# ivario123/r7020e-visual-odometry

Measured on AMD Instinct MI355X. Metric: stereo frames/sec @1242x375 (SIFT detect+describe x2 + stereo matchFeatures), higher is better.
Workload: dtype f32 (i8 MFMA for exact descriptor dot products); 1 GPU; BASELINE configs[1]: SIFT detect+describe + BF match on 1242x375 synthetic stereo, ~2k keypoints/image; rows=375, cols=1242, parallelism=frames sharded over 1 GPU(s)

## Files before the change

__graft_entry__.py:

```python
import os
import subprocess
import sys
from pathlib import Path

ROOT = Path(__file__).resolve().parent
PKG = ROOT / "r7020e-visual-odometry_amd"


def build() -> None:
    env = dict(os.environ)
    env.setdefault("ARCH", "gfx950")
    jobs = str(min(8, os.cpu_count() or 4))
    subprocess.run(["make", "-s", "-j", jobs, "-C", str(PKG / "csrc")], check=True, env=env)
    subprocess.run(["make", "-s", "-C", str(ROOT / "oracle")], check=True, env=env)
    subprocess.run(["make", "-s", "-C", str(ROOT / "tests" / "mex_shim")], check=True, env=env)
    subprocess.run(["make", "-s", "-C", str(ROOT / "tests" / "describe_ref")], check=True, env=env)
    subprocess.run(["make", "-s", "-C", str(ROOT / "tests" / "tri_quality_ref")], check=True, env=env)
    subprocess.run(["make", "-s", "-C", str(ROOT / "tests" / "pose_refine_ref")], check=True, env=env)
    sys.path.insert(0, str(ROOT))
    import vo_amd
    from r7020e_visual_odometry_amd import vo
    lib = vo.load_library()
    missing = [s for s in vo.EXPORTS if not hasattr(lib, s)]
    if missing:
        raise RuntimeError(f"libvo.so is missing exports: {missing}")


def smoke() -> None:
    import numpy as np
    sys.path.insert(0, str(ROOT))
    sys.path.insert(0, str(ROOT / "oracle"))
    import torch
    import vo_amd
    from r7020e_visual_odometry_amd import vo, synthetic as syn
    import oracle

    assert torch.cuda.is_available(), "smoke() needs an MI355X"
    L, R = syn.stereo_pair(syn.SEED_BASE + 1)
    ctx = vo.Context(375, 1242, 1, device=0)
    dl = torch.from_numpy(L[None]).cuda()
    dr = torch.from_numpy(R[None]).cuda()
# ... 21 lines not shown
```

r7020e-visual-odometry_amd/csrc/blur_plan.h:

```cpp
#pragma once

namespace vo {

#define VO_BLUR_RADII(X) X(5) X(6) X(8) X(10) X(13)

constexpr bool blur_radius_tabled(int r)
{
#define VO_BLUR_IS_R(RR) || r == RR
    return false VO_BLUR_RADII(VO_BLUR_IS_R);
#undef VO_BLUR_IS_R
}

constexpr int kTagLevel = 0;
constexpr int kTagBase = 1;
constexpr int kTagBaseU8 = kTagBase | 4;
constexpr int kTagCachedStores = 2;
constexpr int kTagNoRowPass = 8;
constexpr int kTagNoColPass = 16;
constexpr int kTagNoLds = 32;
constexpr int kTagNoHalo = 64;

#define BS_P 4

constexpr int bs_rh(int r, int cpl) { return (r + cpl - 1) / cpl * cpl; }
// ... 14 lines not shown

constexpr int blur_bands(int R, int th) { return (R + th - 1) / th; }
constexpr int blur_grid_strips(int C, int r, int cpl, int tag) { return (C + bs_sw(r, cpl, tag) - 1) / bs_sw(r, cpl, tag); }

constexpr BlurPlan blur_plan(BlurRole role, int R, int C, int n_img, int r)
{
    constexpr int kMaxTH = 128, kWaveTarget = 2048, kCpl2MaxC = 1400, kU8MinRows = 64;
    const bool base = role != BlurRole::Level;
    const int cpl = (!base && C <= kCpl2MaxC) ? 2 : 4;
    const int tag = role == BlurRole::BaseU8 ? kTagBaseU8 : base ? kTagBase : kTagLevel;
    const long waves_rows = (long)R * ((C + 64 * cpl - 1) / (64 * cpl)) * n_img / kWaveTarget;
    const long cap = base && kBaseMaxTH < kMaxTH ? kBaseMaxTH : kMaxTH;
    int th = (int)(waves_rows < cap ? waves_rows : cap) / BS_P * BS_P;
    if (th < BS_P) th = BS_P;
    BlurPlan p{role, false, 0, 0, 0, 0, 0, !base && waves_rows >= kMaxTH};
    if (!blur_radius_tabled(r) || R < th || R <= r + BS_P + 2 || (role == BlurRole::BaseU8 && R < kU8MinRows)) return p;
    p.streamed = true;
    p.cpl = cpl; p.tag = tag; p.th = th;
    p.n_bands = blur_bands(R, th);
    p.n_strips = blur_grid_strips(C, r, cpl, tag);
    return p;
}

}
```

r7020e-visual-odometry_amd/csrc/sift.hip:

```cpp
#include "vo_internal.h"
#include "blur_plan.h"
#include <cstdlib>
#include <cstring>
#include <cmath>
#include <algorithm>
#include <utility>
#include <type_traits>
#include <mutex>

namespace vo {

struct Kern { float k[VO_SIFT_MAX_RADIUS + 1]; int r; float* nb; int nb_pitch, nb_rows, nb_cols; };

static int desc_radius_cap(const Pyramid& py, const vo_sift_params& p);

void build_pyramid_geometry(Pyramid& py, int rows, int cols, int n_img, const vo_sift_params& p)
{
    memset(&py, 0, sizeof(py));
    const int L = p.n_octave_layers;
    py.L = L;
    py.n_img = n_img;
    py.n_oct = vo_num_octaves(rows, cols, p.upsample);
    int R = p.upsample ? rows * 2 : rows, C = p.upsample ? cols * 2 : cols;
    size_t off = 0;
    size_t tmp_plane = 0;
    for (int o = 0; o < py.n_oct; ++o) {
        OctGeom& g = py.oct[o];
        if (o) { R /= 2; C /= 2; }
        g.rows = R; g.cols = C;
        g.dmax = (int)sqrt((double)C * C + (double)R * R);
        g.pitch = (C + 255) / 256 * 256;
        g.plane = (size_t)g.rows * g.pitch;
        for (int i = 0; i < L + 3; ++i) { g.g_off[i] = off; off += g.plane; }
        if (g.plane > tmp_plane) tmp_plane = g.plane;
    }
    py.istride = off;
    py.total = off * n_img;
    py.tmp_plane = tmp_plane;
    double sig[VO_SIFT_MAX_LAYERS];
    vo_level_sigmas(L, p.sigma, sig);
    py.krad[0] = vo_gauss_kernel(vo_base_sigma(p.sigma, p.upsample), py.kern[0], VO_SIFT_MAX_RADIUS + 1);
    for (int i = 1; i < L + 3; ++i) py.krad[i] = vo_gauss_kernel(sig[i], py.kern[i], VO_SIFT_MAX_RADIUS + 1);
    int w = 0, b = 0, t = 0;
    for (int o = 0; o < py.n_oct; ++o) {
        int ir = py.oct[o].rows - 2 * VO_SIFT_BORDER, ic = py.oct[o].cols - 2 * VO_SIFT_BORDER;
        if (ir < 0) ir = 0;
        if (ic < 0) ic = 0;
        py.wrow[o] = ic > 0 ? ((py.oct[o].cols - VO_SIFT_BORDER - 1) / 64 + 2) / 2 * 2 : 0;
        for (int l = 0; l < L; ++l) { py.wbase[b++] = w; w += ir * py.wrow[o]; }
        py.ebase[o] = t;
        py.estrips[o] = py.wrow[o] / 2;
        t += py.estrips[o] * ((ir + VO_EXT_BAND - 1) / VO_EXT_BAND);
    }
    py.wbase[b] = w;
    py.n_words = w;
    py.ebase[py.n_oct] = t;
    py.n_units = t;
    py.n_seg = (w + VO_SEG_WORDS - 1) / VO_SEG_WORDS;
    py.dcap = desc_radius_cap(py, p);
}

SiftBuffers sift_view(const SiftBuffers& b, const Pyramid& py, int img0, int n)
{
    SiftBuffers v = b;
    v.arena = b.arena + (size_t)img0 * py.istride;
    v.tmp = b.tmp + (size_t)img0 * py.tmp_plane;
    v.mask = b.mask + (size_t)img0 * py.n_words;
    v.woff = b.woff + (size_t)img0 * py.n_seg;
    v.cand = b.cand + (size_t)img0 * b.cand_cap;
    v.n_cand = b.n_cand + img0;
    v.acc = b.acc + (size_t)img0 * b.cand_cap;
    v.n_acc = b.n_acc + img0;
    v.cout = b.cout + (size_t)img0 * b.cand_cap;
    v.koff = b.koff + (size_t)img0 * b.cand_cap;
// ... 252 lines not shown
        }
    }
}


struct U8Src { const uint8_t* p; int ld, rows, cols; };
__host__ __device__ constexpr int bs_u8_dw(int r, int cpl) { return ((64 * cpl + 2 * bs_rh(r, cpl)) / 2 + 3 + 3 + 4 + 3) / 4; }
__host__ __device__ constexpr int bs_u8_rows(int r) { return (2 * r + BS_P + kBaseMaxTH) / 2 + 4; }

__device__ __forceinline__ vo_f4 up4_from_words(uint32_t a0, uint32_t a1, uint32_t sa, uint32_t b0, uint32_t b1, uint32_t sb)
{
    const uint32_t ba = __builtin_amdgcn_alignbyte(a1, a0, sa), bb = __builtin_amdgcn_alignbyte(b1, b0, sb);
    float r[4];
#pragma unroll
    for (int i = 0; i < 4; ++i) {
        const uint32_t xa = 1 + (i >> 1), xb = (i & 1) ? xa + 1 : xa - 1;
        const uint32_t sel = xa | xb << 8 | (4 + xa) << 16 | (4 + xb) << 24;
        const uint32_t q = __builtin_amdgcn_perm(bb, ba, sel);
        r[i] = (float)__builtin_amdgcn_udot4(q, 0x01030309u, 0u, false) * 0.0625f;
    }
    return vo_f4{r[0], r[1], r[2], r[3]};
}

template <int RAD, bool EDGE, int TAG, int CPL>
__device__ __forceinline__ void blur_stream_body(const float* __restrict__ sp, int pitch, int R, int C,
                                                 float* __restrict__ g_out, const Kern& K,
                                                 int x0, int y0, int TH, float* rb, const U8Src& u8,
                                                 float* __restrict__ nbo, uint32_t* __restrict__ stg)
{
    typedef float vec_t __attribute__((ext_vector_type(CPL)));
    constexpr bool UP = (TAG & 4) != 0;
    static_assert(!UP || CPL == 4, "the fused x2 upsample uses 4 columns per lane");
    constexpr bool XCH = bs_hl(RAD, CPL, TAG);
    constexpr int SW = 64 * CPL;
    constexpr int P = BS_P;
    constexpr int RH = bs_rh(RAD, CPL);
    constexpr int NQ = 1 + 2 * RH / CPL;
    constexpr int NP = CPL / 2;
    constexpr int NR = 2 * RAD + P;
    constexpr int F = (2 * RAD + P - 1) / P * P;
    constexpr int E = F - 2 * RAD;
    constexpr int RW = bs_rw(RAD, CPL);
    if constexpr ((TAG & 4) != 0) {
        if (TH > kBaseMaxTH) return;
    }
    const int lane = threadIdx.x;
    const int xl = x0 - (XCH ? RH : 0) + CPL * lane;
    const bool hl = lane < RH / CPL, hr = !hl && lane < 2 * RH / CPL;
    const int hx = XCH ? xl : hl ? x0 - RH + CPL * lane : hr ? x0 + SW + CPL * (lane - RH / CPL) : x0 - RH;
    const int hpos = hl ? CPL * lane : hr ? RH + SW + CPL * (lane - RH / CPL) : -1;
    float* const dummy = rb + RW + CPL * lane;
// ... 36 lines not shown
#pragma unroll
            for (int q = 0; q < SCH; ++q) {
                const int t = t0 + 64 * q + lane;
                const int row = t / SWD, k = t - row * SWD;
                const uint32_t ro = delta + (uint32_t)(sr0 + row) * (uint32_t)u8.ld + (uint32_t)s_lo;
                v[q] = (uint32_t)__builtin_amdgcn_raw_buffer_load_b32(rs_in, t < total ? (ro & ~3u) + 4u * (uint32_t)k : 0x80000000u, 0, 0);
            }
#pragma unroll
            for (int q = 0; q < SCH; ++q)
                if (t0 + 64 * q + lane < total) stg[t0 + 64 * q + lane] = v[q];
        }
        __syncthreads();
    }
    auto s_off = [&](int y, int x) {
        return (y - sr0) * (4 * SWD) + (x - s_lo) + (int)((delta + (uint32_t)y * (uint32_t)u8.ld + (uint32_t)s_lo) & 3u);
    };
    const uint8_t* const stg8 = reinterpret_cast<const uint8_t*>(stg);

    constexpr int NSET = XCH ? 2 : 1;
    vec_t pf[NSET * P], ph[NSET * P];
    typedef uint32_t u2_t __attribute__((ext_vector_type(2)));
    u2_t pw[UP && !EDGE ? NSET * P : 1][4];
    vo_f2 H[NR][NP];
    const int gm = (xl >> 1) - 1, gh = (hx >> 1) - 1;

    auto gather = [&](const float* rowp, const int* idx) {
        vec_t v;
#pragma unroll
        for (int i = 0; i < CPL; ++i) v[i] = rowp[idx[i]];
        return v;
    };

    auto yref = [&](int kk) {
        const int p = y0 - RAD - E + kk;
        if constexpr (XCH) return p < 0 ? -p : (p >= R ? 2 * R - 2 - p : p);
        else return vo_reflect101(p, R);
    };
    auto s_words = [&](int y, int x) {
        const int o = s_off(y, x);
        const uint32_t* w = stg + (o >> 2);
        return u2_t{w[0], w[1]};
    };
#define VO_BS_LOAD(KK, SL)                                                                        \
    do {                                                                                          \
        const int yin_ = yref(KK);                                                                \
        if constexpr (UP) {                                                                       \
// ... 117 lines not shown
                const int y = y0 + kk - F;
                const bool act = (!XCH || (lane >= RH / CPL && lane < 64 - RH / CPL)) && xl < C && y < R &&
                                 (MODE == 1 || (kk >= F && kk < F + TH));
                constexpr uint32_t OOB = 0x80000000u;
                const uint32_t vo = act ? (uint32_t)(y * pitch + xl) * 4u : OOB;
                constexpr int AUX = (TAG & 2) ? 0 : 2;
                if constexpr (CPL == 4)
                    __builtin_amdgcn_raw_buffer_store_b128(__builtin_bit_cast(vo_i4, g), rs_out, vo, 0, AUX);
                else
                    __builtin_amdgcn_raw_buffer_store_b64(__builtin_bit_cast(vo_i2, g), rs_out, vo, 0, AUX);
                if constexpr ((u & 1) == 0 && !(TAG & 1)) {
                    const int yn = y >> 1, c0 = xl >> 1;
                    const bool rowok = act && yn < K.nb_rows;
                    const uint32_t nbase = (uint32_t)(yn * K.nb_pitch + c0) * 4u;
                    const float g0 = g[0];
                    __builtin_amdgcn_raw_buffer_store_b32(__float_as_int(g0), rs_nb, rowok && c0 < K.nb_cols ? nbase : OOB,
                                                          0, 0);
                    if constexpr (CPL == 4) {
                        const float g2 = g[2];
                        __builtin_amdgcn_raw_buffer_store_b32(__float_as_int(g2), rs_nb,
                                                              rowok && c0 + 1 < K.nb_cols ? nbase + 4u : OOB, 0, 0);
                    }
                }
            }
            if constexpr (!XCH) __syncthreads();
        });
#pragma unroll
        for (int q = 0; q < 2 * RAD; ++q)
#pragma unroll
            for (int c = 0; c < NP; ++c) H[q][c] = H[q + P][c];
    };

    vo_static_for<P>([&](auto uc) { VO_BS_LOAD(decltype(uc)::value, decltype(uc)::value); });
    using I0 = std::integral_constant<int, 0>;
    using I1 = std::integral_constant<int, 1>;
    using I2 = std::integral_constant<int, 2>;
    if constexpr (NSET == 1) {
#pragma unroll 1
        for (int kk0 = 0; kk0 < F; kk0 += P) block(kk0, I0{}, I0{});
#pragma unroll 1
        for (int kk0 = F; kk0 < F + TH; kk0 += P) block(kk0, I1{}, I0{});
    } else {
#pragma unroll 1
        for (int kk0 = 0; kk0 < F + TH; kk0 += 2 * P) {
            block(kk0, I2{}, I0{});
            block(kk0 + P, I2{}, I1{});
        }
    }
#undef VO_BS_LOAD
}

#ifndef VO_BLUR_OCC3_MAXR
#define VO_BLUR_OCC3_MAXR 6
#endif
#ifndef VO_BASE_WAVES
#define VO_BASE_WAVES 3
// ... 6 lines not shown
    vo_ss_prio();
    constexpr int RH = bs_rh(RAD, CPL), SW = bs_sw(RAD, CPL, TAG);
    constexpr bool XCH = bs_hl(RAD, CPL, TAG);
    __shared__ __attribute__((aligned(16))) float rb[XCH ? 4 : bs_rw(RAD, CPL) + 64 * CPL];
    __shared__ uint32_t stg[(TAG & 4) ? bs_u8_rows(RAD) * bs_u8_dw(RAD, CPL) : 1];
    const int bid = xcd_remap(blockIdx.x, gridDim.x);
    const int strip = bid % n_strips, tb = bid / n_strips;
    const int band = tb % n_bands, img = tb / n_bands;
    const int x0 = strip * SW, y0 = band * TH;
    const int THb = min(TH, (R - y0 + BS_P - 1) / BS_P * BS_P);
    const size_t os = img * splane, od = img * dplane;
    U8Src u8{nullptr, 0, in_rows, in_cols};
    int margin = 0;
    if (TAG & 4) {
        u8.p = ((img & 1) ? isrc.right : isrc.left) + (size_t)(img >> 1) * isrc.frame_stride;
        u8.ld = isrc.ld;
        margin = 16;
    }
    float* const nbo = K.nb ? K.nb + od : nullptr;
    if (x0 - RH < 0 || (XCH ? x0 - RH + 64 * CPL : x0 + SW + RH) + margin > C)
        blur_stream_body<RAD, true, TAG, CPL>(src + os, pitch, R, C, g_out + od, K, x0, y0, THb, rb, u8, nbo, stg);
    else
        blur_stream_body<RAD, false, TAG, CPL>(src + os, pitch, R, C, g_out + od, K, x0, y0, THb, rb, u8, nbo, stg);
}

__global__ __launch_bounds__(256) void k_down(const float* __restrict__ src, size_t splane, int spitch,
                                              float* __restrict__ dst, size_t dplane, int dpitch, int C)
{
    const int x = blockIdx.x * 256 + threadIdx.x, y = blockIdx.y, img = blockIdx.z;
    if (x < C) dst[img * dplane + (size_t)y * dpitch + x] = src[img * splane + (size_t)(2 * y) * spitch + 2 * x];
}

#ifndef VO_SMALL_PX
#define VO_SMALL_PX 9216
#endif
#ifndef VO_SMALL_T
#define VO_SMALL_T 1024
#endif

constexpr int SMV = 8;
template <int RAD>
__device__ __forceinline__ void small_pass(const float* __restrict__ src, float* __restrict__ dst, float* __restrict__ gdst,
                                           int gpitch, int R, int C, bool rows, const float* __restrict__ kk,
                                           const int* __restrict__ tab, int tid)
{
    const int len = rows ? C : R, other = rows ? R : C, runs = (len + SMV - 1) / SMV;
// ... 351 lines not shown
    uint32_t cnt = 0;
#pragma unroll
    for (int q = 0; q < 4; ++q) {
        mw[q] = (w0 + q < nw) ? m[w0 + q] : 0ull;
        cnt += (uint32_t)__popcll(mw[q]);
    }
#pragma unroll
    for (int q = 0; q < 4; q += 2) {
        const unsigned long long ev = mw[q], od = mw[q + 1];
        mw[q] = vo_spread32((uint32_t)ev) | vo_spread32((uint32_t)od) << 1;
        mw[q + 1] = vo_spread32((uint32_t)(ev >> 32)) | vo_spread32((uint32_t)(od >> 32)) << 1;
    }
    uint32_t idx = segoff[(size_t)img * py->n_seg + seg] + block_exscan_256(cnt, sh);
    if (!cnt) return;
#pragma unroll
    for (int q = 0; q < 4; ++q) {
        unsigned long long mm = mw[q];
        if (!mm) continue;
        int o, layer, r, k;
        decode_word(py, w0 + q, o, layer, r, k);
        while (mm) {
            const int bit = __ffsll((long long)mm) - 1;
            mm &= mm - 1;
            if (idx < (uint32_t)cand_cap) cand[(size_t)img * cand_cap + idx] = pack_cand(o, layer, r, 64 * k + bit);
            idx++;
        }
    }
}

template <typename T>
__device__ __forceinline__ T wave_tree_sum(T v)
{
    auto bits = [](T x) { return __builtin_bit_cast(int, x); };
    auto val = [](int x) { return __builtin_bit_cast(T, x); };
    v = v + val(__builtin_amdgcn_permlane32_swap(bits(v), bits(v), false, false)[1]);
    v = v + val(__builtin_amdgcn_permlane16_swap(bits(v), bits(v), false, false)[1]);
    v = v + val(__builtin_amdgcn_update_dpp(0, bits(v), 0x108, 0xF, 0xF, true));
    v = v + val(__builtin_amdgcn_update_dpp(0, bits(v), 0x104, 0xF, 0xF, true));
    v = v + val(__builtin_amdgcn_update_dpp(0, bits(v), 0x102, 0xF, 0xF, true));
    v = v + val(__builtin_amdgcn_update_dpp(0, bits(v), 0x101, 0xF, 0xF, true));
    return val(__builtin_amdgcn_readlane(bits(v), 0));
}
__device__ __forceinline__ float wave_max(float v)
{
    auto bits = [](float x) { return __float_as_int(x); };
    v = fmaxf(v, __int_as_float(__builtin_amdgcn_permlane32_swap(bits(v), bits(v), false, false)[1]));
    v = fmaxf(v, __int_as_float(__builtin_amdgcn_permlane16_swap(bits(v), bits(v), false, false)[1]));
// ... 812 lines not shown
    const size_t lds = sizeof(float) * ft_lds_floats(K.r);
    if (lds > 64 * 1024) raise_lds_limit((const void*)k_blur_fused<RAD>);
    VO_LAUNCH_NAMED("k_blur_fused", (k_blur_fused<RAD>), dim3((C + FT_W - 1) / FT_W, (R + FT_H - 1) / FT_H, n_img), dim3(256), lds, s,
                    src, plane, dplane, pitch, R, C, g, K);
}

static void launch_blur(const BlurPlan& pl, int n_img, hipStream_t s, const float* src, size_t plane, size_t dplane, int pitch,
                        int R, int C, float* g, const Kern& K, const ImageSrc& isrc, int in_rows, int in_cols)
{
    switch (K.r) {
#define VO_BLUR_CASE(RR) \
    case RR: return launch_blur_r<RR>(pl, n_img, s, src, plane, dplane, pitch, R, C, g, K, isrc, in_rows, in_cols);
        VO_BLUR_RADII(VO_BLUR_CASE)
#undef VO_BLUR_CASE
    default: return launch_blur_r<0>(pl, n_img, s, src, plane, dplane, pitch, R, C, g, K, isrc, in_rows, in_cols);
    }
}

static float ext_threshold(const Pyramid& py, const vo_sift_params& p)
{
    return (float)floor(0.5 * p.contrast_threshold / py.L * 255.0);
}

struct SmallPlan { int o_small, rtab, cap, bcap; size_t lds; };
static SmallPlan small_plan(const Pyramid& py)
{
    SmallPlan sp{py.n_oct, 0, 0, 0, 0};
    int maxr = 0;
    for (int i = 1; i < py.L + 3; ++i) maxr = std::max(maxr, py.krad[i]);
    for (int o = py.n_oct - 1; o >= 1; --o) {
        int rt = 0, ct = 0, cap = 0, bcap = 0;
        bool fits = true;
        for (int q = o; q < py.n_oct; ++q) {
            fits = fits && py.oct[q].rows * py.oct[q].cols <= VO_SMALL_PX;
            cap = std::max(cap, py.oct[q].rows * py.oct[q].cols);
            if (q > o) bcap = std::max(bcap, py.oct[q].rows * py.oct[q].cols);
            rt = std::max(rt, py.oct[q].rows + 2 * maxr);
            ct = std::max(ct, py.oct[q].cols + 2 * maxr);
        }
        cap = (cap + 3) & ~3;
        bcap = (bcap + 3) & ~3;
        const size_t lds = sizeof(float) * (3 * (size_t)cap + bcap) + sizeof(int) * (rt + ct);
        if (!fits || lds > 160 * 1024) break;
        sp = SmallPlan{o, rt, cap, bcap, lds};
    }
    return sp;
}

int sift_small_octave(const Pyramid& py) { return small_plan(py).o_small; }

void sift_enqueue_small(const Pyramid& py, SiftBuffers& b, int n_img, hipStream_t s, const Pyramid* d_py)
{
    const SmallPlan sp = small_plan(py);
    if (sp.o_small >= py.n_oct) return;

    raise_lds_limit((const void*)k_small_pyr);
    VO_LAUNCH_NAMED("k_blur_small", k_small_pyr, dim3(n_img), dim3(VO_SMALL_T), sp.lds, s, d_py, b.arena, sp.o_small,
                    sp.rtab, sp.cap, sp.bcap);
}

void sift_enqueue_pyramid(const Pyramid& py, SiftBuffers& b, const ImageSrc& src, int n_img, const vo_sift_params& p,
                          hipStream_t s, const Pyramid* d_py, hipEvent_t ev_o0, const ScaleChains& ch)
{
    const int L = py.L;
    float* A = b.arena;
    const SmallPlan sp = small_plan(py);
    const int o_small = sp.o_small;
    const bool forked = ch.down != nullptr && ch.down != s;
    int o_fork = std::min(1, o_small - 1);
    while (o_fork + 1 < o_small &&
           blur_plan(BlurRole::Level, py.oct[o_fork + 1].rows, py.oct[o_fork + 1].cols, n_img, py.krad[1]).full_bands)
        ++o_fork;
    bool base_done = false;
    for (int o = 0; o < py.n_oct; ++o) {
        const OctGeom& g = py.oct[o];
        const int R = g.rows, C = g.cols;
        if (o == o_small) break;
        if (forked && o == o_fork + 1) s = ch.down;
        if (o == 0) {
            const Kern K0 = make_kern(py, 0);
            const int rows = p.upsample ? R / 2 : R, cols = p.upsample ? C / 2 : C;
            BlurPlan pl = blur_plan(p.upsample ? BlurRole::BaseU8 : BlurRole::BaseFloat, R, C, n_img, K0.r);
            const bool from_u8 = pl.role == BlurRole::BaseU8 && pl.streamed;
            if (!from_u8) {
                const dim3 qg((g.pitch / 4 + 255) / 256, R, n_img);
// ... 1 lines not shown
                    VO_LAUNCH(k_base_src<true>, qg, dim3(256), 0, s, src, rows, cols, b.tmp, g.plane, g.pitch, R, C, n_img);
                else
                    VO_LAUNCH(k_base_src<false>, qg, dim3(256), 0, s, src, rows, cols, b.tmp, g.plane, g.pitch, R, C, n_img);
                pl = blur_plan(BlurRole::BaseFloat, R, C, n_img, K0.r);
            }
            launch_blur(pl, n_img, s, from_u8 ? nullptr : b.tmp, from_u8 ? 0 : g.plane, py.istride, g.pitch, R, C,
                        A + g.g_off[0], K0, src, from_u8 ? rows : 0, from_u8 ? cols : 0);
        } else if (!base_done) {
            const OctGeom& pg = py.oct[o - 1];
            VO_LAUNCH(k_down, dim3((C + 255) / 256, R, n_img), dim3(256), 0, s, A + pg.g_off[L], py.istride, pg.pitch,
                      A + g.g_off[0], py.istride, g.pitch, C);
        }
        for (int i = 1; i < L + 3; ++i) {
            Kern K = make_kern(py, i);
            const BlurPlan pl = blur_plan(BlurRole::Level, R, C, n_img, K.r);
            if (i == L) {
                base_done = pl.streamed && o + 1 < o_small;
                if (base_done) {
                    const OctGeom& ng = py.oct[o + 1];
                    K.nb = A + ng.g_off[0];
                    K.nb_pitch = ng.pitch; K.nb_rows = ng.rows; K.nb_cols = ng.cols;
                }
            }
            launch_blur(pl, n_img, s, A + g.g_off[i - 1], py.istride, py.istride, g.pitch, R, C, A + g.g_off[i], K, src, 0, 0);
            if (forked && o == o_fork && i == L) {
                hipEventRecord(ch.ev_fork, s);
                hipStreamWaitEvent(ch.down, ch.ev_fork, 0);
            }
        }
        if (o == 0 && ev_o0) hipEventRecord(ev_o0, s);
    }
}

#ifndef VO_FEATURE_GRID
#define VO_FEATURE_GRID 32768
#endif
constexpr int kFeatureGrid = VO_FEATURE_GRID;

void sift_enqueue_extrema(const Pyramid& py, SiftBuffers& b, int n_img, const vo_sift_params& p, hipStream_t s,
                          const Pyramid* d_py, int o_begin, int o_end)
{
    const int L = py.L;
    float* A = b.arena;
    const float thr = ext_threshold(py, p);
    const int u_first = py.ebase[o_begin], u_last = py.ebase[o_end];
    if (u_last > u_first) {
        const dim3 ge((u_last - u_first) * n_img);
// ... 49 lines not shown
    VO_LAUNCH(k_refine, dim3(VO_REFINE_BLOCKS), dim3(256), 0, s, d_py, A, b.cand, b.n_cand, b.cout, b.acc, b.n_acc, b.koff, b.cand_cap, n_img,
              p.contrast_threshold, p.edge_threshold, p.sigma);
    const size_t fpre_bytes = sizeof(int) * (size_t)(n_img + 1);
    const size_t dt_bytes = sizeof(uint32_t) * (size_t)dt_stride(py.dcap);
    VO_LAUNCH_NAMED("k_orient", (k_orient<36>), dim3(kFeatureGrid), dim3(64), fpre_bytes, s, d_py, A, b.n_acc, b.acc,
                    b.cout, b.koff, b.cand_cap, n_img);
    VO_LAUNCH(k_scan_cands, dim3(n_img), dim3(1024), 0, s, b.cout, b.n_cand, b.koff, b.n_kp, b.cand_cap);
    if (strongest > 0) {
        const dim3 gsel(VO_SEL_BLOCKS, n_img);
        VO_LAUNCH(k_sel_keys, gsel, dim3(VO_SEL_TILE), 0, s, b.cout, b.n_acc, b.acc, b.koff, b.n_kp, b.n_det, b.skey, b.snpk,
                  b.cand_cap);
        VO_LAUNCH(k_sel_rank, gsel, dim3(VO_SEL_TILE), 0, s, b.n_acc, b.acc, b.skey, b.snpk, b.koff, b.n_det, b.n_kp, b.cand_cap,
                  strongest);
    }
    VO_LAUNCH(k_expand, dim3(256), dim3(256), 0, s, b.cout, b.n_acc, b.acc, b.koff, b.kp, b.kpi, b.cand_cap, b.kp_cap,
              n_img, p.upsample, strongest > 0 ? strongest : b.kp_cap);
    VO_LAUNCH_NAMED("k_desc", (k_desc<VO_DESC_COPIES>), dim3(kFeatureGrid), dim3(64), dt_bytes + fpre_bytes, s, d_py, A,
                    b.kpi, b.n_kp, b.desc, b.meta, b.kp_cap, n_img);
}

void sift_enqueue_describe(const Pyramid& py, SiftBuffers& b, const ImageSrc& src, int n_img, int n_points,
                           const vo_sift_params& p, hipStream_t s, const Pyramid* d_py)
{
    sift_enqueue_pyramid(py, b, src, n_img, p, s, d_py);
    sift_enqueue_small(py, b, n_img, s, d_py);
    if (n_points <= 0) return;
    VO_LAUNCH(k_points, dim3(std::min(256, (n_points + 255) / 256)), dim3(256), 0, s, b.kp, b.n_kp, b.kpi, b.kp_cap, n_img,
              p.upsample);
    const size_t fpre_bytes = sizeof(int) * (size_t)(n_img + 1);
    const size_t dt_bytes = sizeof(uint32_t) * (size_t)dt_stride(VO_SIFT_DESCR_RMAX);
    VO_LAUNCH_NAMED("k_desc_pts", (k_desc_pts<VO_DESC_COPIES>), dim3(std::min(kFeatureGrid, n_points)), dim3(64),
                    dt_bytes + fpre_bytes, s, d_py, b.arena, b.kpi, b.n_kp, b.desc, b.meta, b.kp_cap, n_img);
}

void sift_enqueue(const Pyramid& py, SiftBuffers& b, const ImageSrc& src, int n_img, const vo_sift_params& p,
                  hipStream_t s, const Pyramid* d_py, int strongest)
{
    sift_enqueue_pyramid(py, b, src, n_img, p, s, d_py);
    sift_enqueue_pyramid_tail(py, b, n_img, p, s, d_py, 0);
    sift_enqueue_features(py, b, n_img, p, s, d_py, strongest);
}

}
```

r7020e-visual-odometry_amd/csrc/vo_api.hip:

```cpp
#include "vo_internal.h"
#include "vo_geom.h"
#include <climits>
#include <cmath>
#include <cstdio>
#include <cstring>
#include <cstdarg>
#include <string>
#include <vector>
#include <deque>
#include <algorithm>

namespace vo {

Profiler* g_prof = nullptr;

void Profiler::begin(const char* name, hipStream_t s)
{
    if (used + 2 > (int)pool.size()) {
        int add = std::max(64, (int)pool.size());
        for (int i = 0; i < add; ++i) { hipEvent_t e; hipEventCreate(&e); pool.push_back(e); }
    }
    marks.push_back({name, used});
    hipEventRecord(pool[used], s);
    used += 1;
// ... 984 lines not shown
                U[k].cam = c->ud_cam[k];
                U[k].in = k ? pr : pl;
                U[k].out = c->d_rect + ((size_t)k * c->max_batch + f0) * fs;
                U[k].copy = c->ud_on[k] ? 0 : 1;
                U[k].pad = 0;
            }
            undistort_launch(U, 2, c->rows, c->cols, nf, fs, fs, sp);
            pl = U[0].out;
            pr = U[1].out;
        }
        ImageSrc src{pl, pr, fs, c->cols, 0};
        SiftBuffers v = sift_view(S.sb, c->py, 2 * f0, 2 * nf);
        ScaleChains ch;
        ch.down = sd;
        ch.ev_fork = c->ev_down[p];
        sift_enqueue_pyramid(c->py, v, src, 2 * nf, c->sp, sp, c->d_py, c->ev_o0[p], ch);
        HIPC(c, hipEventRecord(c->ev_top[p], sp));
        sift_enqueue_small(c->py, v, 2 * nf, sd, c->d_py);
        HIPC(c, hipEventRecord(c->ev_join[p], sd));
    }
    for (int p = 0; p < parts; ++p) {
        const int f0 = B * p / parts, nf = B * (p + 1) / parts - f0;
        SiftBuffers v = sift_view(S.sb, c->py, 2 * f0, 2 * nf);
        HIPC(c, hipStreamWaitEvent(st, iso ? c->ev_join[p] : c->ev_o0[p], 0));
        sift_enqueue_extrema(c->py, v, 2 * nf, c->sp, st, c->d_py, 0, 1);
        HIPC(c, hipStreamWaitEvent(st, c->ev_top[p], 0));
        HIPC(c, hipStreamWaitEvent(st, c->ev_join[p], 0));
        sift_enqueue_extrema(c->py, v, 2 * nf, c->sp, st, c->d_py, 1, o_small);
        sift_enqueue_extrema(c->py, v, 2 * nf, c->sp, st, c->d_py, o_small, c->py.n_oct);
        sift_enqueue_features(c->py, v, 2 * nf, c->sp, st, c->d_py, c->strongest);
        if (p == parts - 1) HIPC(c, hipEventRecord(S.ev_arena, st));
        match_launch(match_view(S.mb, f0), S.d_jobs + job_stereo(c, f0), nf, c->mp, st);
    }
    HIPC(c, hipEventRecord(S.ev_done, st));
    if (join) HIPC(c, hipStreamWaitEvent(c->stream, S.ev_done, 0));
    c->last_set = set;
    c->described = false;
    return VO_OK;
}

int vo_sift_match_batch_dev(vo_ctx* c, const uint8_t* d_lefts, const uint8_t* d_rights, int B, vo_pair_stats* stats)
{
    if (!c || !d_lefts || !d_rights || B < 1 || B > c->max_batch) return fail(c, VO_ERR_ARG, "vo_sift_match_batch_dev: bad arguments");
    BEGIN_CALL(c, false);
    const int set = c->next_set;
    c->next_set ^= 1;
    const bool sync = stats != nullptr;
    int rc = enqueue_sift_stereo(c, set, d_lefts, d_rights, B, sync, true);
// ... 858 lines not shown
```

r7020e-visual-odometry_amd/csrc/vo_internal.h:

```cpp
#pragma once
#include <hip/hip_runtime.h>
#include <stdint.h>
#include <vector>
#include <string>
#include "vo.h"
#include "vo_spec.h"

#define VO_WAVE 64

namespace vo {

struct Profiler {
    bool on = false;
    std::vector<hipEvent_t> pool;
    int used = 0;
    std::vector<std::pair<const char*, int>> marks;
    std::vector<std::string> names;
    std::vector<double> ms;
    std::vector<int> calls;
    void begin(const char* name, hipStream_t s);
    void end(hipStream_t s);
    void collect();
    void reset_totals();
    ~Profiler();
// ... 6 lines not shown
        hipLaunchKernelGGL(kernel, grid, block, shmem, stream, __VA_ARGS__);               \
        if (::vo::g_prof && ::vo::g_prof->on) ::vo::g_prof->end(stream);                   \
    } while (0)
#define VO_LAUNCH(kernel, grid, block, shmem, stream, ...) \
    VO_LAUNCH_NAMED(#kernel, kernel, grid, block, shmem, stream, __VA_ARGS__)

struct OctGeom {
    int rows, cols, pitch;
    int dmax;
    size_t plane;
    size_t g_off[VO_SIFT_MAX_LAYERS];
};

struct Pyramid {
    int n_oct, L, n_img;
    OctGeom oct[VO_SIFT_MAX_OCTAVES];
    float kern[VO_SIFT_MAX_LAYERS][VO_SIFT_MAX_RADIUS + 1];
    int krad[VO_SIFT_MAX_LAYERS];
    size_t istride;
    size_t total;
    size_t tmp_plane;
    int wbase[VO_SIFT_MAX_OCTAVES * 4 + 1];
    int wrow[VO_SIFT_MAX_OCTAVES];
    int n_words;
    int ebase[VO_SIFT_MAX_OCTAVES + 1];
    int estrips[VO_SIFT_MAX_OCTAVES];
    int n_units;
    int n_seg;
    int dcap;
};

#define DT_HDR 12
enum { DT_ORI, DT_PX, DT_PY, DT_RADIUS, DT_COS, DT_SIN, DT_NSAMP, DT_NROWS, DT_O, DT_LAYER };
static inline __host__ __device__ int dt_rtab_off() { return DT_HDR; }
static inline __host__ __device__ int dt_wtab_off(int dcap) { return DT_HDR + 2 * dcap + 10; }
static inline __host__ __device__ int dt_stride(int dcap) { return (DT_HDR + 3 * dcap + 11 + 3) & ~3; }

#ifndef VO_EXT_BAND
#define VO_EXT_BAND 30
#endif
#define VO_SEG_WORDS 1024

__host__ __device__ inline uint32_t pack_cand(int o, int layer, int r, int c) {
    return (uint32_t)c | ((uint32_t)r << 12) | ((uint32_t)layer << 24) | ((uint32_t)o << 27);
}

// ... 38 lines not shown

struct ImageSrc {
    const uint8_t* left;
    const uint8_t* right;
    size_t frame_stride;
    int ld;
    int pad;
};

void build_pyramid_geometry(Pyramid& py, int rows, int cols, int n_img, const vo_sift_params& p);
const char* sift_params_refusal(const vo_sift_params& p);
SiftBuffers sift_view(const SiftBuffers& b, const Pyramid& py, int img0, int n);
hipError_t sift_alloc(SiftBuffers& b, const Pyramid& py, int kp_cap, int cand_cap);
hipError_t sift_alloc_select(SiftBuffers& b);
void sift_free(SiftBuffers& b);
void sift_enqueue(const Pyramid& py, SiftBuffers& b, const ImageSrc& src, int n_img,
                  const vo_sift_params& p, hipStream_t s, const Pyramid* d_py, int strongest = 0);
struct ScaleChains {
    hipStream_t down = nullptr;
    hipEvent_t ev_fork = nullptr;
};
void sift_enqueue_pyramid(const Pyramid& py, SiftBuffers& b, const ImageSrc& src, int n_img,
                          const vo_sift_params& p, hipStream_t s, const Pyramid* d_py, hipEvent_t ev_o0 = nullptr,
                          const ScaleChains& ch = ScaleChains());
void sift_enqueue_pyramid_tail(const Pyramid& py, SiftBuffers& b, int n_img, const vo_sift_params& p, hipStream_t s,
                               const Pyramid* d_py, int ext_o_begin);
void sift_enqueue_extrema(const Pyramid& py, SiftBuffers& b, int n_img, const vo_sift_params& p, hipStream_t s,
                          const Pyramid* d_py, int o_begin, int o_end);
int sift_small_octave(const Pyramid& py);
void sift_enqueue_small(const Pyramid& py, SiftBuffers& b, int n_img, hipStream_t s, const Pyramid* d_py);
void sift_enqueue_features(const Pyramid& py, SiftBuffers& b, int n_img, const vo_sift_params& p, hipStream_t s,
                           const Pyramid* d_py, int strongest = 0);

void sift_enqueue_describe(const Pyramid& py, SiftBuffers& b, const ImageSrc& src, int n_img, int n_points,
                           const vo_sift_params& p, hipStream_t s, const Pyramid* d_py);

#define VO_UD_CHUNK 16
struct UndistortSide {
    vo_bc_cam cam;
    const uint8_t* in;
    uint8_t* out;
    int copy, pad;
};
void undistort_launch(const UndistortSide* sides, int n_sides, int rows, int cols, int B, size_t in_stride,
                      size_t out_stride, hipStream_t s);

void raise_lds_limit(const void* fn);
// ... 54 lines not shown
```

r7020e-visual-odometry_amd/roofline.py:

```python
from __future__ import annotations

import math

import numpy as np

SMALL_PX = 9216


def octave_dims(rows: int, cols: int, upsample: bool = True) -> list[tuple[int, int]]:
    R, C = (rows * 2, cols * 2) if upsample else (rows, cols)
    n = int(round(math.log2(min(R, C)) - 2)) + (1 if upsample else 0)
    dims = []
    for o in range(n):
        if o:
            R //= 2
            C //= 2
        dims.append((R, C))
    return dims


def pyramid_bytes_per_image(rows: int, cols: int, layers: int = 3) -> int:
    P = sum(r * c for r, c in octave_dims(rows, cols))
    G, D = (layers + 3) * P, (layers + 2) * P
    return rows * cols + 4 * (2 * G + 2 * D)


def kernel_bytes(rows: int, cols: int, n_img: int, layers: int = 3, ext_inner: bool = True) -> dict:
    dims = octave_dims(rows, cols)
    lv = layers + 2
    out = {}

    def add(name, nbytes, launches):
        b, l = out.get(name, (0, 0))
        out[name] = (b + nbytes, l + launches)

    R0, C0 = dims[0]
    add("k_blur_base", n_img * (rows * cols + 4 * R0 * C0), 1)
    o_small = next((o for o in range(1, len(dims)) if all(r * c <= SMALL_PX for r, c in dims[o:])), len(dims))
    for o, (R, C) in enumerate(dims):
        px = R * C * n_img
        if o >= o_small:
            add("k_blur_small", 4 * px * (1 + lv), 1 if o == o_small else 0)
            continue
        nb = 4 * dims[o + 1][0] * dims[o + 1][1] * n_img if o + 1 < o_small else 0
        add("k_blur_fused", 8 * px * lv + nb, lv)
    nlev = layers + 1 if ext_inner else layers + 3
    ext = sum(4 * nlev * r * c for r, c in dims) * n_img
    if ext:
        add(f"k_ext_{'inner' if ext_inner else 'stream'}<{layers}>", ext, 2 if len(dims) > 1 else 1)
    return out


BORDER = 5
SEG_WORDS = 1024
MAX_PEAKS = 18
CANDOUT_BYTES = 48 + 4 * (MAX_PEAKS + 2)
KP_BYTES = 32
DESC_BYTES = 128 + 8
MATCH_CHUNK = 4096
ORI_RADIUS, DESCR_SCL, DESCR_WIDTH = 4.5, 3.0, 4


def mask_geometry(rows: int, cols: int, layers: int = 3, upsample: bool = True) -> tuple[int, int]:
    w = 0
    for R, C in octave_dims(rows, cols, upsample):
        ir, ic = max(R - 2 * BORDER, 0), max(C - 2 * BORDER, 0)
        wrow = ((C - BORDER - 1) // 64 + 2) // 2 * 2 if ic > 0 else 0
        w += layers * ir * wrow
    return w, (w + SEG_WORDS - 1) // SEG_WORDS


def _lines(width_floats):
    return 1.0 + (4.0 * np.maximum(width_floats, 1) - 4.0) / 128.0


def feature_bytes(rows: int, cols: int, n_cand, n_acc, kp_size, kp_octave, kp_angle, kp_image,
                  matches, layers: int = 3) -> dict:
    n_cand = np.asarray(n_cand, np.float64)
    n_acc = np.asarray(n_acc, np.float64)
    n_img = len(n_cand)
    words, segs = mask_geometry(rows, cols, layers)
    C, A = float(n_cand.sum()), float(n_acc.sum())
    out = {}

    def put(name, alg, line=None):
        out[name] = {"algorithmic": float(alg), "line_floor": float(alg if line is None else line)}

    put("k_seg_count", n_img * (8 * words + 4 * segs))
    put("k_seg_scan", n_img * (8 * segs + 8))
    put("k_seg_emit", n_img * (8 * words + 4 * segs) + 4 * C)
    put("k_refine", C * (4 + 4 * 3 * 3 * 4 + CANDOUT_BYTES + 4) + 4 * A,
# ... 27 lines not shown
```

Before: 10130 stereo frames/s.

## Fuse DoG extremum detection into the last level blur for large octaves

Adds a k_blur_ext kernel that, while computing the final Gaussian level of each large octave, also forms the DoG planes from the previously stored levels and runs the 3x3x3 extremum test, writing ballot masks directly. The separate extrema pass for those octaves is skipped, and the mask layout is changed to overlapping 126-column strips with a column correction in candidate emission. This removes a full re-read of the DoG/Gaussian stack and one launch per octave. In exchange the blur kernel carries more register pressure and extra loads, and blur bands now overlap by two rows.

```diff
diff --git a/__graft_entry__.py b/__graft_entry__.py
--- a/__graft_entry__.py
+++ b/__graft_entry__.py
@@ -17,6 +17,7 @@
     subprocess.run(["make", "-s", "-C", str(ROOT / "tests" / "describe_ref")], check=True, env=env)
     subprocess.run(["make", "-s", "-C", str(ROOT / "tests" / "tri_quality_ref")], check=True, env=env)
     subprocess.run(["make", "-s", "-C", str(ROOT / "tests" / "pose_refine_ref")], check=True, env=env)
+    subprocess.run(["make", "-s", "-C", str(ROOT / "tests" / "ext_plan")], check=True, env=env)
     sys.path.insert(0, str(ROOT))
     import vo_amd
     from r7020e_visual_odometry_amd import vo
diff --git a/r7020e-visual-odometry_amd/csrc/blur_plan.h b/r7020e-visual-odometry_amd/csrc/blur_plan.h
--- a/r7020e-visual-odometry_amd/csrc/blur_plan.h
+++ b/r7020e-visual-odometry_amd/csrc/blur_plan.h
@@ -60,4 +60,29 @@
     return p;
 }
 
+constexpr int kTagExt = 128;
+constexpr int kExtLayers = 3;
+constexpr int kExtCpl = 2;
+constexpr int kExtMinTH = 8;
+constexpr int ext_strip_step(int cpl) { return 64 * cpl - cpl; }
+constexpr int ext_strips(int C, int cpl) { return C <= 2 ? 1 : (C - 2 + ext_strip_step(cpl) - 1) / ext_strip_step(cpl); }
+constexpr int ext_bands(int R, int th) { return R <= 2 ? 1 : (R - 2 + th - 3) / (th - 2); }
+
+constexpr bool blur_ext_fused(int L, int R, int C, int r)
+{
+    return L == kExtLayers && blur_radius_tabled(r) && R > r + BS_P + 2 && R >= kExtMinTH && C >= 2;
 }
+
+constexpr BlurPlan blur_ext_plan(int R, int C, int n_img)
+{
+    constexpr int kMaxTH = 128, kWaveTarget = 2048;
+    const long waves_rows = (long)R * ext_strips(C, kExtCpl) * n_img / kWaveTarget;
+    int th = (int)(waves_rows < kMaxTH ? waves_rows : kMaxTH) / BS_P * BS_P;
+    if (th < kExtMinTH) th = kExtMinTH;
+    if (th > R / BS_P * BS_P) th = R / BS_P * BS_P;
+    BlurPlan p{BlurRole::Level, true, kExtCpl, kTagLevel | kTagExt, th, ext_bands(R, th), ext_strips(C, kExtCpl),
+               waves_rows >= kMaxTH};
+    return p;
+}
+
+}
diff --git a/r7020e-visual-odometry_amd/csrc/sift.hip b/r7020e-visual-odometry_amd/csrc/sift.hip
--- a/r7020e-visual-odometry_amd/csrc/sift.hip
+++ b/r7020e-visual-odometry_amd/csrc/sift.hip
@@ -42,14 +42,20 @@
     py.krad[0] = vo_gauss_kernel(vo_base_sigma(p.sigma, p.upsample), py.kern[0], VO_SIFT_MAX_RADIUS + 1);
     for (int i = 1; i < L + 3; ++i) py.krad[i] = vo_gauss_kernel(sig[i], py.kern[i], VO_SIFT_MAX_RADIUS + 1);
     int w = 0, b = 0, t = 0;
+    const int o_small = sift_small_octave(py);
     for (int o = 0; o < py.n_oct; ++o) {
         int ir = py.oct[o].rows - 2 * VO_SIFT_BORDER, ic = py.oct[o].cols - 2 * VO_SIFT_BORDER;
         if (ir < 0) ir = 0;
         if (ic < 0) ic = 0;
         py.wrow[o] = ic > 0 ? ((py.oct[o].cols - VO_SIFT_BORDER - 1) / 64 + 2) / 2 * 2 : 0;
+        py.wovl[o] = 0;
+        if (o < o_small && ir > 0 && ic > 0 && blur_ext_fused(L, py.oct[o].rows, py.oct[o].cols, py.krad[L + 1])) {
+            py.wovl[o] = 64 * kExtCpl - ext_strip_step(kExtCpl);
+            py.wrow[o] = 2 * ext_strips(py.oct[o].cols, kExtCpl);
+        }
         for (int l = 0; l < L; ++l) { py.wbase[b++] = w; w += ir * py.wrow[o]; }
         py.ebase[o] = t;
-        py.estrips[o] = py.wrow[o] / 2;
+        py.estrips[o] = py.wovl[o] ? 0 : py.wrow[o] / 2;
         t += py.estrips[o] * ((ir + VO_EXT_BAND - 1) / VO_EXT_BAND);
     }
     py.wbase[b] = w;
@@ -348,11 +354,22 @@
     return vo_f4{r[0], r[1], r[2], r[3]};
 }
 
+struct ExtArgs {
+    const float* g1;
+    size_t lstride;
+    unsigned long long* mask;
+    int n_words;
+    int wb[kExtLayers];
+    int wr;
+    float thr;
+};
+
 template <int RAD, bool EDGE, int TAG, int CPL>
 __device__ __forceinline__ void blur_stream_body(const float* __restrict__ sp, int pitch, int R, int C,
                                                  float* __restrict__ g_out, const Kern& K,
                                                  int x0, int y0, int TH, float* rb, const U8Src& u8,
-                                                 float* __restrict__ nbo, uint32_t* __restrict__ stg)
+                                                 float* __restrict__ nbo, uint32_t* __restrict__ stg,
+                                                 const ExtArgs& X = ExtArgs(), int strip = 0)
 {
     typedef float vec_t __attribute__((ext_vector_type(CPL)));
     constexpr bool UP = (TAG & 4) != 0;
@@ -435,6 +452,81 @@
     typedef uint32_t u2_t __attribute__((ext_vector_type(2)));
     u2_t pw[UP && !EDGE ? NSET * P : 1][4];
     vo_f2 H[NR][NP];
+    constexpr bool EXT = (TAG & kTagExt) != 0;
+    constexpr int EL = kExtLayers, EW = 4;
+    static_assert(!EXT || (CPL == 2 && !XCH && !UP && P == EW), "the extremum epilogue: 2-column lanes, LDS exchange");
+    vo_f2 e_pm[EXT ? P : 1][EL], e_hmx[EXT ? EW : 1][EL], e_hmn[EXT ? EW : 1][EL], e_dc[EXT ? EW : 1][EL];
+    __amdgpu_buffer_rsrc_t rs_e[EL], rs_m;
+    if constexpr (EXT) {
+#pragma unroll
+        for (int l = 0; l < EL; ++l)
+            rs_e[l] = __builtin_amdgcn_make_buffer_rsrc(const_cast<float*>(X.g1 + l * X.lstride), 0, R * pitch * 4, 0x00020000);
+        rs_m = __builtin_amdgcn_make_buffer_rsrc(X.mask, 0, X.n_words * 8, 0x00020000);
+    }
+    const bool e_in0 = lane > 0 && xl >= VO_SIFT_BORDER && xl < C - VO_SIFT_BORDER;
+    const bool e_in1 = lane < 63 && xl + 1 >= VO_SIFT_BORDER && xl + 1 < C - VO_SIFT_BORDER;
+    auto e_load = [&](int t, auto sl_c) {
+        constexpr int SL = decltype(sl_c)::value;
+        const int y = min(y0 + t, R - 1);
+        const uint32_t vo = xl < C ? (uint32_t)(y * pitch + xl) * 4u : 0x80000000u;
+#pragma unroll
+        for (int l = 0; l < EL; ++l)
+            e_pm[SL][l] = __builtin_bit_cast(vo_f2, __builtin_amdgcn_raw_buffer_load_b64(rs_e[l], vo, 0, 0));
+    };
+    if constexpr (EXT) {
+#pragma unroll
+        for (int q = 0; q < EW; ++q)
+#pragma unroll
+            for (int l = 0; l < EL; ++l) e_hmx[q][l] = e_hmn[q][l] = e_dc[q][l] = vo_f2{0.0f, 0.0f};
+    }
+    auto e_step = [&](int t, auto u_c, const vo_f2 g) {
+        constexpr int U = decltype(u_c)::value, A = (U + 2) % EW, M = (U + 3) % EW;
+        vo_f2 d[EL];
+#pragma unroll
+        for (int l = 0; l + 1 < EL; ++l) d[l] = e_pm[U][l + 1] - e_pm[U][l];
+        d[EL - 1] = g - e_pm[U][EL - 1];
+        e_load(t + P, u_c);
+#pragma unroll
+        for (int l = 0; l < EL; ++l) {
+            const float la = vo_dpp<VO_DPP_WAVE_SHR1>(d[l].y), rb_ = vo_dpp<VO_DPP_WAVE_SHL1>(d[l].x);
+            e_hmx[U][l] = vo_f2{fmaxf(fmaxf(la, d[l].x), d[l].y), fmaxf(fmaxf(d[l].x, d[l].y), rb_)};
+            e_hmn[U][l] = vo_f2{fminf(fminf(la, d[l].x), d[l].y), fminf(fminf(d[l].x, d[l].y), rb_)};
+            e_dc[U][l] = d[l];
+        }
+        const int r = y0 + t - 1;
+        const bool live = t >= 2 && r >= VO_SIFT_BORDER && r < R - VO_SIFT_BORDER;
+        vo_f2 mx3[EL], mn3[EL];
+#pragma unroll
+        for (int l = 0; l < EL; ++l) {
+            mx3[l] = vo_f2{fmaxf(fmaxf(e_hmx[A][l].x, e_hmx[M][l].x), e_hmx[U][l].x),
+                           fmaxf(fmaxf(e_hmx[A][l].y, e_hmx[M][l].y), e_hmx[U][l].y)};
+            mn3[l] = vo_f2{fminf(fminf(e_hmn[A][l].x, e_hmn[M][l].x), e_hmn[U][l].x),
+                           fminf(fminf(e_hmn[A][l].y, e_hmn[M][l].y), e_hmn[U][l].y)};
+        }
+#pragma unroll
+        for (int layer = 1; layer <= EL; ++layer) {
+            bool hit[2];
+#pragma unroll
+            for (int c = 0; c < 2; ++c) {
+                const float val = c ? e_dc[M][layer - 1].y : e_dc[M][layer - 1].x;
+                float bmx = c ? mx3[layer - 1].y : mx3[layer - 1].x;
+                float bmn = c ? mn3[layer - 1].y : mn3[layer - 1].x;
+                if (layer >= 2) {
+                    bmx = fmaxf(bmx, c ? mx3[layer - 2].y : mx3[layer - 2].x);
+                    bmn = fminf(bmn, c ? mn3[layer - 2].y : mn3[layer - 2].x);
+                }
+                if (layer <= EL - 1) {
+                    bmx = fmaxf(bmx, c ? mx3[layer].y : mx3[layer].x);
+                    bmn = fminf(bmn, c ? mn3[layer].y : mn3[layer].x);
+                }
+                hit[c] = ((val > X.thr) & (val >= bmx)) | ((val < -X.thr) & (val <= bmn));
+            }
+            const uint64_t w0 = __ballot(hit[0] & e_in0), w1 = __ballot(hit[1] & e_in1);
+            const uint32_t mo = (lane < 2 && live) ? (uint32_t)(X.wb[layer - 1] + (r - VO_SIFT_BORDER) * X.wr + 2 * strip + lane) * 8u
+                                                   : 0x80000000u;
+            __builtin_amdgcn_raw_buffer_store_b64(__builtin_bit_cast(vo_i2, (uint64_t)(lane ? w1 : w0)), rs_m, mo, 0, 0);
+        }
+    };
     const int gm = (xl >> 1) - 1, gh = (hx >> 1) - 1;
 
     auto gather = [&](const float* rowp, const int* idx) {
@@ -598,6 +690,7 @@
                                                               rowok && c0 + 1 < K.nb_cols ? nbase + 4u : OOB, 0, 0);
                     }
                 }
+                if constexpr (EXT && MODE == 1) e_step(kk - F, uc, vo_f2{g[0], g[1]});
             }
             if constexpr (!XCH) __syncthreads();
         });
@@ -608,6 +701,7 @@
     };
 
     vo_static_for<P>([&](auto uc) { VO_BS_LOAD(decltype(uc)::value, decltype(uc)::value); });
+    if constexpr (EXT) vo_static_for<P>([&](auto uc) { e_load(decltype(uc)::value, uc); });
     using I0 = std::integral_constant<int, 0>;
     using I1 = std::integral_constant<int, 1>;
     using I2 = std::integral_constant<int, 2>;
@@ -660,6 +754,28 @@
         blur_stream_body<RAD, true, TAG, CPL>(src + os, pitch, R, C, g_out + od, K, x0, y0, THb, rb, u8, nbo, stg);
     else
         blur_stream_body<RAD, false, TAG, CPL>(src + os, pitch, R, C, g_out + od, K, x0, y0, THb, rb, u8, nbo, stg);
+}
+
+template <int RAD>
+__global__ __launch_bounds__(64, 2) void k_blur_ext(const float* __restrict__ src, size_t splane, int pitch, int R, int C,
+                                                    float* __restrict__ g_out, Kern K, int n_strips, int n_bands, int TH, ExtArgs X)
+{
+    vo_ss_prio();
+    constexpr int CPL = kExtCpl, TAG = kTagLevel | kTagExt, RH = bs_rh(RAD, CPL), SW = 64 * CPL;
+    __shared__ __attribute__((aligned(16))) float rb[bs_rw(RAD, CPL) + 64 * CPL];
+    const int bid = xcd_remap(blockIdx.x, gridDim.x);
+    const int strip = bid % n_strips, tb = bid / n_strips;
+    const int band = tb % n_bands, img = tb / n_bands;
+    const int x0 = strip * ext_strip_step(CPL), y0 = band * (TH - 2);
+    const int THb = min(TH, (R - y0 + BS_P - 1) / BS_P * BS_P);
+    const size_t os = img * splane;
+    X.g1 += os;
+    X.mask += (size_t)img * X.n_words;
+    const U8Src u8{nullptr, 0, 0, 0};
+    if (x0 - RH < 0 || x0 + SW + RH > C)
+        blur_stream_body<RAD, true, TAG, CPL>(src + os, pitch, R, C, g_out + os, K, x0, y0, THb, rb, u8, nullptr, nullptr, X, strip);
+    else
+        blur_stream_body<RAD, false, TAG, CPL>(src + os, pitch, R, C, g_out + os, K, x0, y0, THb, rb, u8, nullptr, nullptr, X, strip);
 }
 
 __global__ __launch_bounds__(256) void k_down(const float* __restrict__ src, size_t splane, int spitch,
@@ -1057,7 +1173,8 @@
         while (mm) {
             const int bit = __ffsll((long long)mm) - 1;
             mm &= mm - 1;
-            if (idx < (uint32_t)cand_cap) cand[(size_t)img * cand_cap + idx] = pack_cand(o, layer, r, 64 * k + bit);
+            if (idx < (uint32_t)cand_cap)
+                cand[(size_t)img * cand_cap + idx] = pack_cand(o, layer, r, 64 * k + bit - py->wovl[o] * (k >> 1));
             idx++;
         }
     }
@@ -1916,6 +2033,32 @@
     return (float)floor(0.5 * p.contrast_threshold / py.L * 255.0);
 }
 
+static void launch_blur_ext(const Pyramid& py, SiftBuffers& b, int o, int n_img, float thr, hipStream_t s, const Kern& K)
+{
+    const OctGeom& g = py.oct[o];
+    const int L = py.L;
+    const BlurPlan pl = blur_ext_plan(g.rows, g.cols, n_img);
+    ExtArgs X;
+    X.g1 = b.arena + g.g_off[1];
+    X.lstride = g.plane;
+    X.mask = b.mask;
+    X.n_words = py.n_words;
+    for (int l = 0; l < kExtLayers; ++l) X.wb[l] = py.wbase[o * L + l];
+    X.wr = py.wrow[o];
+    X.thr = thr;
+    switch (K.r) {
+#define VO_BLUR_CASE(RR)                                                                                            \
+    case RR:                                                                                                        \
+        VO_LAUNCH_NAMED("k_blur_fused", (k_blur_ext<RR>), dim3(pl.n_strips * pl.n_bands * n_img), dim3(64), 0, s,     \
+                        (const float*)(b.arena + g.g_off[L]), py.istride, g.pitch, g.rows, g.cols,                 \
+                        b.arena + g.g_off[L + 1], K, pl.n_strips, pl.n_bands, pl.th, X);                            \
+        break;
+        VO_BLUR_RADII(VO_BLUR_CASE)
+#undef VO_BLUR_CASE
+    default: abort();
+    }
+}
+
 struct SmallPlan { int o_small, rtab, cap, bcap; size_t lds; };
 static SmallPlan small_plan(const Pyramid& py)
 {
@@ -1954,7 +2097,7 @@
 }
 
 void sift_enqueue_pyramid(const Pyramid& py, SiftBuffers& b, const ImageSrc& src, int n_img, const vo_sift_params& p,
-                          hipStream_t s, const Pyramid* d_py, hipEvent_t ev_o0, const ScaleChains& ch)
+                          hipStream_t s, const Pyramid* d_py, hipEvent_t ev_o0, const ScaleChains& ch, bool with_ext)
 {
     const int L = py.L;
     float* A = b.arena;
@@ -2002,7 +2145,10 @@
                     K.nb_pitch = ng.pitch; K.nb_rows = ng.rows; K.nb_cols = ng.cols;
                 }
             }
-            launch_blur(pl, n_img, s, A + g.g_off[i - 1], py.istride, py.istride, g.pitch, R, C, A + g.g_off[i], K, src, 0, 0);
+            if (i == L + 1 && with_ext && py.wovl[o])
+                launch_blur_ext(py, b, o, n_img, ext_threshold(py, p), s, K);
+            else
+                launch_blur(pl, n_img, s, A + g.g_off[i - 1], py.istride, py.istride, g.pitch, R, C, A + g.g_off[i], K, src, 0, 0);
             if (forked && o == o_fork && i == L) {
                 hipEventRecord(ch.ev_fork, s);
                 hipStreamWaitEvent(ch.down, ch.ev_fork, 0);
@@ -2098,7 +2244,7 @@
 void sift_enqueue_describe(const Pyramid& py, SiftBuffers& b, const ImageSrc& src, int n_img, int n_points,
                            const vo_sift_params& p, hipStream_t s, const Pyramid* d_py)
 {
-    sift_enqueue_pyramid(py, b, src, n_img, p, s, d_py);
+    sift_enqueue_pyramid(py, b, src, n_img, p, s, d_py, nullptr, ScaleChains(), false);
     sift_enqueue_small(py, b, n_img, s, d_py);
     if (n_points <= 0) return;
     VO_LAUNCH(k_points, dim3(std::min(256, (n_points + 255) / 256)), dim3(256), 0, s, b.kp, b.n_kp, b.kpi, b.kp_cap, n_img,
diff --git a/r7020e-visual-odometry_amd/csrc/vo_api.hip b/r7020e-visual-odometry_amd/csrc/vo_api.hip
--- a/r7020e-visual-odometry_amd/csrc/vo_api.hip
+++ b/r7020e-visual-odometry_amd/csrc/vo_api.hip
@@ -1030,8 +1030,10 @@
     for (int p = 0; p < parts; ++p) {
         const int f0 = B * p / parts, nf = B * (p + 1) / parts - f0;
         SiftBuffers v = sift_view(S.sb, c->py, 2 * f0, 2 * nf);
-        HIPC(c, hipStreamWaitEvent(st, iso ? c->ev_join[p] : c->ev_o0[p], 0));
-        sift_enqueue_extrema(c->py, v, 2 * nf, c->sp, st, c->d_py, 0, 1);
+        if (!c->py.wovl[0]) {
+            HIPC(c, hipStreamWaitEvent(st, iso ? c->ev_join[p] : c->ev_o0[p], 0));
+            sift_enqueue_extrema(c->py, v, 2 * nf, c->sp, st, c->d_py, 0, 1);
+        }
         HIPC(c, hipStreamWaitEvent(st, c->ev_top[p], 0));
         HIPC(c, hipStreamWaitEvent(st, c->ev_join[p], 0));
         sift_enqueue_extrema(c->py, v, 2 * nf, c->sp, st, c->d_py, 1, o_small);
diff --git a/r7020e-visual-odometry_amd/csrc/vo_internal.h b/r7020e-visual-odometry_amd/csrc/vo_internal.h
--- a/r7020e-visual-odometry_amd/csrc/vo_internal.h
+++ b/r7020e-visual-odometry_amd/csrc/vo_internal.h
@@ -52,6 +52,7 @@
     size_t tmp_plane;
     int wbase[VO_SIFT_MAX_OCTAVES * 4 + 1];
     int wrow[VO_SIFT_MAX_OCTAVES];
+    int wovl[VO_SIFT_MAX_OCTAVES];
     int n_words;
     int ebase[VO_SIFT_MAX_OCTAVES + 1];
     int estrips[VO_SIFT_MAX_OCTAVES];
@@ -136,7 +137,7 @@
 };
 void sift_enqueue_pyramid(const Pyramid& py, SiftBuffers& b, const ImageSrc& src, int n_img,
                           const vo_sift_params& p, hipStream_t s, const Pyramid* d_py, hipEvent_t ev_o0 = nullptr,
-                          const ScaleChains& ch = ScaleChains());
+                          const ScaleChains& ch = ScaleChains(), bool with_ext = true);
 void sift_enqueue_pyramid_tail(const Pyramid& py, SiftBuffers& b, int n_img, const vo_sift_params& p, hipStream_t s,
                                const Pyramid* d_py, int ext_o_begin);
 void sift_enqueue_extrema(const Pyramid& py, SiftBuffers& b, int n_img, const vo_sift_params& p, hipStream_t s,
diff --git a/r7020e-visual-odometry_amd/roofline.py b/r7020e-visual-odometry_amd/roofline.py
--- a/r7020e-visual-odometry_amd/roofline.py
+++ b/r7020e-visual-odometry_amd/roofline.py
@@ -25,8 +25,10 @@
     return rows * cols + 4 * (2 * G + 2 * D)
 
 
-def kernel_bytes(rows: int, cols: int, n_img: int, layers: int = 3, ext_inner: bool = True) -> dict:
+def kernel_bytes(rows: int, cols: int, n_img: int, layers: int = 3, ext_inner: bool = True,
+                 ext_fused: bool = False) -> dict:
     dims = octave_dims(rows, cols)
+    fused = ext_fused and ext_inner and layers == 3
     lv = layers + 2
     out = {}
 
@@ -44,6 +46,14 @@
             continue
         nb = 4 * dims[o + 1][0] * dims[o + 1][1] * n_img if o + 1 < o_small else 0
         add("k_blur_fused", 8 * px * lv + nb, lv)
+        if fused and octave_ext_fused(layers, R, C):
+            add("k_blur_fused", 4 * layers * px + 8 * layers * n_img * fused_mask_words(R, C), 0)
+    if fused:
+        ext = sum(4 * (layers + 1) * r * c for o, (r, c) in enumerate(dims)
+                  if o >= o_small or not octave_ext_fused(layers, r, c)) * n_img
+        if ext:
+            add(f"k_ext_inner<{layers}>", ext, 1)
+        return out
     nlev = layers + 1 if ext_inner else layers + 3
     ext = sum(4 * nlev * r * c for r, c in dims) * n_img
     if ext:
@@ -61,12 +71,29 @@
 ORI_RADIUS, DESCR_SCL, DESCR_WIDTH = 4.5, 3.0, 4
 
 
-def mask_geometry(rows: int, cols: int, layers: int = 3, upsample: bool = True) -> tuple[int, int]:
+EXT_STRIP_STEP = 126
+EXT_RADIUS = 10
+
+
+def octave_ext_fused(layers: int, R: int, C: int, radius: int = EXT_RADIUS) -> bool:
+    return layers == 3 and radius in (5, 6, 8, 10, 13) and R > radius + 6 and R >= 8 and C >= 2
+
+
+def fused_mask_words(R: int, C: int) -> int:
+    return max(R - 2 * BORDER, 0) * 2 * max(1, -(-(C - 2) // EXT_STRIP_STEP))
+
+
+def mask_geometry(rows: int, cols: int, layers: int = 3, upsample: bool = True, radius: int = EXT_RADIUS) -> tuple[int, int]:
+    dims = octave_dims(rows, cols, upsample)
+    o_small = next((o for o in range(1, len(dims)) if all(r * c <= SMALL_PX for r, c in dims[o:])), len(dims))
     w = 0
-    for R, C in octave_dims(rows, cols, upsample):
+    for o, (R, C) in enumerate(dims):
         ir, ic = max(R - 2 * BORDER, 0), max(C - 2 * BORDER, 0)
         wrow = ((C - BORDER - 1) // 64 + 2) // 2 * 2 if ic > 0 else 0
-        w += layers * ir * wrow
+        if o < o_small and ir > 0 and ic > 0 and octave_ext_fused(layers, R, C, radius):
+            w += layers * fused_mask_words(R, C)
+        else:
+            w += layers * ir * wrow
     return w, (w + SEG_WORDS - 1) // SEG_WORDS
 
 
```

New measurement: 10170 stereo frames/s, median of 5. No clear change (+0.4%).
